# HpWang-whu/RoReg

Measured on AMD Instinct MI355X. Metric: pair-registrations/sec, higher is better.
Workload: dtype f32 (every f32 operand enters the fp16 matrix cores as hi + lo fp16 under a per-keypoint power-of-two block scale: <= 22 significant bits relative to a CONSERVATIVE per-keypoint bound -- measured on the extractor: the bound sits 2^2..2^6 above the keypoint's true coefficient maximum (config.f16x2_sc

## Files before the change

roreg_amd/csrc/fourier.hip:

```cpp
#include "common.h"
#include "primitives.h"
#include <algorithm>
#include <atomic>
#include <cmath>
#include <cstdlib>
#include <type_traits>
#include <utility>
#include <vector>

namespace {

constexpr int NIRR = 5;

struct GemmDescs {
    const float *X[NIRR];
    float *Out[NIRR];
    const float *Add[NIRR];
    const float4 *W[NIRR];
    int K[NIRR], M[NIRR], Mpad[NIRR], N[NIRR];
};

template <int CT>
__global__ __launch_bounds__(256, 2) void irrep_gemm_kernel(GemmDescs p, const int *__restrict__ tiles) {
    extern __shared__ __attribute__((aligned(16))) char smem[];
// ... 1576 lines not shown
    const float *A1, *A2;
    const bf16x8 *A1s, *A2s;
    const f16x8 *A1h, *A2h;
    int f_exp;
    const float *out_bound;
    float *out_rowmax;
    int x_bf16;
    int out_planes;
    int sp_pack;
    float *raw_col;
    int raw_g;
    int B, Bp, C, tiles_per_c, Lout, Lvalid;
    const roreg::LtRow *g_rows;
    const int64_t *g_dr;
    const uint8_t *g_P8;
};

struct QRows { int alpha[64], d[64], i[64]; };
constexpr QRows make_qrows() {
    QRows t{};
    const int dims[NIRR] = {1, 3, 3, 4, 5};
    int off = 0, q = 0;
    for (int r = 0; r < NIRR; ++r) {
        for (int i = 0; i < dims[r]; ++i)
            for (int l = 0; l < dims[r]; ++l, ++q) { t.alpha[q] = off + l * dims[r]; t.d[q] = dims[r]; t.i[q] = i; }
        off += dims[r] * dims[r];
    }
    for (; q < 64; ++q) { t.alpha[q] = 0; t.d[q] = 1; t.i[q] = 0; }
    return t;
}
constexpr QRows kQ = make_qrows();

struct PairSlots {
    int qa[32], qb[32];
    int row[32];
    int i[32];
    int kind[32];
    int d[32];
    int row_alpha[16], row_d[16];
};
constexpr PairSlots make_pair_slots() {
    PairSlots t{};
    const int dims[NIRR] = {1, 3, 3, 4, 5};
    int off = 0, s = 0, row0 = 0;
    for (int r = 0; r < NIRR; ++r) {
        const int d = dims[r];
        for (int l = 0; l < d; ++l) {
            t.row_alpha[row0 + l] = off + l * d; t.row_d[row0 + l] = d;
            for (int i = d % 2; i < d; i += 2, ++s) {
                t.qa[s] = off + i * d + l; t.qb[s] = off + (i + 1) * d + l; t.row[s] = row0 + l; t.i[s] = i; t.kind[s] = 0; t.d[s] = d;
            }
        }
        if (d % 2)
            for (int l = 0; l < d; l += 2, ++s) {
                t.qa[s] = off + l; t.row[s] = row0 + l; t.i[s] = 0; t.d[s] = d;
                if (l + 1 < d) { t.qb[s] = off + l + 1; t.kind[s] = 1; } else { t.qb[s] = 64; t.kind[s] = 2; }
            }
        off += d * d; row0 += d;
    }
    return t;
}
constexpr PairSlots kPS = make_pair_slots();
constexpr int slot_out_q(int m) { const int mm = m & 31, s = (m >> 5) * 16 + (mm & 3) + 4 * (mm >> 3); return (mm & 4) ? kPS.qb[s] : kPS.qa[s]; }

template <int... I, class F>
__device__ __forceinline__ void static_for_impl(std::integer_sequence<int, I...>, F &&f) { (f(std::integral_constant<int, I>{}), ...); }
template <int N, class F>
__device__ __forceinline__ void static_for(F &&f) { static_for_impl(std::make_integer_sequence<int, N>{}, f); }

template <bool IN_SPATIAL, bool OUT_SPATIAL, int SPLIT , int NW , int MINW , bool OUT_ROWS = false, bool GATHER = false >
__global__ __launch_bounds__(NW * 64, MINW) void ft_nonlin_kernel(NonlinParams p) {
    constexpr int NT = NW * 64;
    const int lane = threadIdx.x & 63;
    const int jn = lane & 31, h = lane >> 5;
    const int wave_global = __builtin_amdgcn_readfirstlane((blockIdx.x * NT + threadIdx.x) >> 6);
    const int n_waves = gridDim.x * NW;
    const int B = p.B, C = p.C;
    const int n_tiles = C * p.tiles_per_c;

    constexpr int NPL = SPLIT == 2 ? 2 : 3;
    constexpr int NA1 = SPLIT ? 4 * 2 * NPL * 64 * 4 : 30 * 2 * 64, NA2 = SPLIT ? 4 * 2 * NPL * 64 * 4 : 32 * 2 * 64;
    __shared__ __attribute__((aligned(16))) float sA1[IN_SPATIAL ? 64 : NA1];
    __shared__ __attribute__((aligned(16))) float sA2[OUT_SPATIAL ? 64 : NA2];
    __shared__ float sT[(IN_SPATIAL || OUT_SPATIAL || OUT_ROWS) ? NW * 32 * 65 : 64];
    {
        const float *g1 = SPLIT == 3 ? reinterpret_cast<const float *>(p.A1s) : SPLIT == 2 ? reinterpret_cast<const float *>(p.A1h) : p.A1;
        const float *g2 = SPLIT == 3 ? reinterpret_cast<const float *>(p.A2s) : SPLIT == 2 ? reinterpret_cast<const float *>(p.A2h) : p.A2;
        if (!IN_SPATIAL)
            for (int i = threadIdx.x; i < NA1; i += NT) sA1[i] = g1[i];
        if (!OUT_SPATIAL)
            for (int i = threadIdx.x; i < NA2; i += NT) sA2[i] = g2[i];
    }
    __shared__ float sBias[512], sScale[512], sShift[512];
    __shared__ int sGmap[64];
    if (threadIdx.x < 64) sGmap[threadIdx.x] = (OUT_SPATIAL && p.g_map && threadIdx.x < ROREG_G) ? p.g_map[threadIdx.x] : (int)threadIdx.x;
    __shared__ uint8_t sP8[GATHER ? ROREG_G * ROREG_G : 4];
    if constexpr (GATHER)
        for (int i = threadIdx.x; i < ROREG_G * ROREG_G; i += NT) sP8[i] = p.g_P8[i];
    for (int i = threadIdx.x; i < p.C; i += NT) {
        sBias[i] = (p.bias ? p.bias[i] : 0.f) + (p.bias2 ? p.bias2[i] : 0.f);
        sScale[i] = p.bn_scale ? p.bn_scale[i] : 1.f;
        sShift[i] = p.bn_shift ? p.bn_shift[i] : 0.f;
    }
    __syncthreads();
    const bf16x8 *sA1s = reinterpret_cast<const bf16x8 *>(sA1), *sA2s = reinterpret_cast<const bf16x8 *>(sA2);
    const f16x8 *sA1h = reinterpret_cast<const f16x8 *>(sA1), *sA2h = reinterpret_cast<const f16x8 *>(sA2);
    const size_t Bp = (size_t)p.Bp;
    const size_t hmask = (size_t)0 - (size_t)h;
#define OFF_Q(Q, c, tb) ((size_t)(kQ.alpha[Q] * C + (c) * kQ.d[Q]) * Bp + (size_t)(tb) * (32 * kQ.d[Q]) + kQ.i[Q] * 32)
#define OFF_OF(Q0, Q1, c, tb) (OFF_Q(Q0, c, tb) + ((OFF_Q(Q1, c, tb) - OFF_Q(Q0, c, tb)) & hmask))
    const unsigned lane_next = (unsigned)lane * 4u;
    const unsigned lane_row3 = (unsigned)jn * 4u + (h ? 12u * (unsigned)C * (unsigned)p.Bp : 0u);
    const unsigned lane_row5 = (unsigned)jn * 4u + (h ? 20u * (unsigned)C * (unsigned)p.Bp : 0u);
    auto row_off = [&](auto rc, int c, int tb) -> size_t {
        constexpr int R = decltype(rc)::value;
        return ((size_t)(kPS.row_alpha[R] * C) + (size_t)(c * kPS.row_d[R])) * Bp + (size_t)tb * (32 * kPS.row_d[R]);
    };
    auto slot_ptr = [&](auto sc, const void *buf, int c, int tb) -> const char * {
        constexpr int S = decltype(sc)::value;
        const char *rb = reinterpret_cast<const char *>(buf) + 4 * row_off(std::integral_constant<int, kPS.row[S]>{}, c, tb) + 128 * kPS.i[S];
        return rb + (kPS.kind[S] == 1 ? (kPS.d[S] == 3 ? lane_row3 : lane_row5) : lane_next);
    };

    constexpr int NCV = IN_SPATIAL ? 32 : (SPLIT != 0 ? 32 : 30);
    constexpr bool PACK_OUT = SPLIT == 2 && !OUT_SPATIAL && !OUT_ROWS;
    auto ld_sp = [&](const float *base, size_t i) -> float {
        return p.x_bf16 ? __uint_as_float((unsigned)reinterpret_cast<const unsigned short *>(base)[i] << 16) : base[i];
    };
    float cn[NCV + 1];
    struct GDesc { unsigned lo, hi; int a; };
    auto load_desc = [&](int tile) -> GDesc {
        GDesc d{0u, 0u, 0};
        if constexpr (GATHER) {
            const int c = tile % C, tb = tile / C;
            const int row = min(tb * 32 + jn, B - 1);
            const uint2 w = *reinterpret_cast<const uint2 *>(&p.g_rows[row].src[c >> 5]);
            d.lo = w.x; d.hi = w.y;
            d.a = reinterpret_cast<const int *>(p.g_dr)[2 * (size_t)row];
        }
        return d;
    };
    auto load_rows_gathered = [&](int tile, const GDesc &d, float (&dst)[NCV + 1]) {
        if constexpr (GATHER) {
            const int c = tile % C, tb = tile / C;
            if constexpr (PACK_OUT) dst[NCV] = p.out_bound[tb * 32 + jn];
            const int cg = (c & 31) * ROREG_G, ln = lane < ROREG_G ? lane : 0;
            const bool permuted = !((c >> 5) & 1);
            auto rows = [&](auto bf16c, auto permc) {
                static_for<32>([&](auto ic) {
                    constexpr int i = decltype(ic)::value;
                    const unsigned long long base = ((unsigned long long)(unsigned)__builtin_amdgcn_readlane((int)d.hi, i) << 32) |
                                                    (unsigned)__builtin_amdgcn_readlane((int)d.lo, i);
                    int g = ln;
                    if constexpr (decltype(permc)::value) g = sP8[__builtin_amdgcn_readlane(d.a, i) * ROREG_G + ln];
                    if constexpr (decltype(bf16c)::value)
                        dst[i] = __uint_as_float(lane < ROREG_G ? (unsigned)reinterpret_cast<const unsigned short *>(base)[cg + g] : 0u);
                    else
                        dst[i] = lane < ROREG_G ? reinterpret_cast<const float *>(base)[cg + g] : 0.f;
                });
            };
            using T_ = std::true_type; using F_ = std::false_type;
            if (p.x_bf16) { if (permuted) rows(T_{}, T_{}); else rows(T_{}, F_{}); }
            else { if (permuted) rows(F_{}, T_{}); else rows(F_{}, F_{}); }
        }
    };
    auto load_coefs = [&](int tile, float (&dst)[NCV + 1]) {
        const int c = (IN_SPATIAL || OUT_SPATIAL) ? tile % C : tile / p.tiles_per_c;
        const int tb = (IN_SPATIAL || OUT_SPATIAL) ? tile / C : tile - c * p.tiles_per_c;
        if constexpr (PACK_OUT) dst[NCV] = p.out_bound[tb * 32 + jn];
        if constexpr (OUT_SPATIAL && SPLIT == 2) { if (p.sp_pack) dst[NCV] = p.out_bound[tb * 32 + jn]; }
        if constexpr (IN_SPATIAL) {
            const int b0 = tb * 32;
            if (p.x_bf16) {
                const unsigned short *xs16 = reinterpret_cast<const unsigned short *>(p.x_spatial);
                static_for<32>([&](auto ic) {
                    constexpr int i = decltype(ic)::value;
                    const size_t src = ((size_t)(b0 + i < B ? b0 + i : B - 1) * C + c) * ROREG_G;
                    dst[i] = __uint_as_float(lane < ROREG_G ? (unsigned)xs16[src + lane] : 0u);
                });
            } else {
                static_for<32>([&](auto ic) {
                    constexpr int i = decltype(ic)::value;
                    const size_t src = ((size_t)(b0 + i < B ? b0 + i : B - 1) * C + c) * ROREG_G;
                    dst[i] = lane < ROREG_G ? p.x_spatial[src + lane] : 0.f;
                });
            }
        } else if constexpr (SPLIT != 0) {
            static_for<32>([&](auto ic) {
                constexpr int st = decltype(ic)::value / 8, e = decltype(ic)::value % 8;
                constexpr int q0 = 16 * st + e, q1 = 16 * st + 8 + e;
                if constexpr (q1 < ROREG_G) dst[st * 8 + e] = __builtin_nontemporal_load(p.Xin + OFF_OF(q0, q1, c, tb) + jn);
                else dst[st * 8 + e] = __builtin_nontemporal_load(p.Xin + OFF_Q(q0, c, tb) + jn);
            });
        } else {
            static_for<30>([&](auto ic) {
                constexpr int s = decltype(ic)::value;
                constexpr int q0 = 2 * s, q1 = 2 * s + 1;
                dst[s] = p.Xin[OFF_OF(q0, q1, c, tb) + jn];
            });
        }
    };
    auto mfma6 = [&](const bf16x8 *a, const bf16x8 &b1, const bf16x8 &b2, const bf16x8 &b3, f32x16 c) {
        const bf16x8 a1 = a[0], a2 = a[64], a3 = a[128];
        c = __builtin_amdgcn_mfma_f32_32x32x16_bf16(a3, b1, c, 0, 0, 0);
        c = __builtin_amdgcn_mfma_f32_32x32x16_bf16(a2, b2, c, 0, 0, 0);
        c = __builtin_amdgcn_mfma_f32_32x32x16_bf16(a1, b3, c, 0, 0, 0);
        c = __builtin_amdgcn_mfma_f32_32x32x16_bf16(a2, b1, c, 0, 0, 0);
        c = __builtin_amdgcn_mfma_f32_32x32x16_bf16(a1, b2, c, 0, 0, 0);
        c = __builtin_amdgcn_mfma_f32_32x32x16_bf16(a1, b1, c, 0, 0, 0);
        return c;
    };
    auto mfma3 = [&](const f16x8 *a, const f16x8 &bh, const f16x8 &bl, f32x16 c) {
        const f16x8 ah = a[0], al = a[64];
        c = __builtin_amdgcn_mfma_f32_32x32x16_f16(al, bh, c, 0, 0, 0);
        c = __builtin_amdgcn_mfma_f32_32x32x16_f16(ah, bl, c, 0, 0, 0);
        c = __builtin_amdgcn_mfma_f32_32x32x16_f16(ah, bh, c, 0, 0, 0);
        return c;
    };
    auto column_scale = [&](float mx, float &xscale, float &oscale) {
        mx = fmaxf(mx, __shfl_xor(mx, 32));
        int e = 0;
        if (mx > 0.f && mx < __builtin_inff()) { int ex; (void)frexpf(mx, &ex); e = 14 - ex; }
        xscale = ldexpf(1.f, e); oscale = ldexpf(1.f, -(e + p.f_exp));
    };
    auto process = [&](int tile, int next_tile, float (&cv)[NCV + 1], float (&cnext)[NCV + 1], int next2_tile, const GDesc &dnext, GDesc &dnext2) {
        asm volatile("" ::: "memory");
        const int c = (IN_SPATIAL || OUT_SPATIAL) ? tile % C : tile / p.tiles_per_c;
        const int tbi = (IN_SPATIAL || OUT_SPATIAL) ? tile / C : tile - c * p.tiles_per_c;
        const int b = tbi * 32 + jn;
        const bool valid = b < B;
        const int bb = valid ? b : B - 1;
        f32x16 v[2];
        float wmax = 0.f;
        if (IN_SPATIAL) {
            if constexpr (GATHER) {
                dnext2 = load_desc(next2_tile);
                load_rows_gathered(next_tile, dnext, cnext);
            } else {
                load_coefs(next_tile, cnext);
            }
            __builtin_amdgcn_sched_barrier(0);
            float *ti = sT + (threadIdx.x >> 6) * (32 * 65);
#pragma unroll
            for (int i = 0; i < 32; ++i) ti[i * 65 + lane] = p.x_bf16 ? __uint_as_float(__float_as_uint(cv[i]) << 16) : cv[i];
            asm volatile("s_waitcnt lgkmcnt(0)" ::: "memory");
#pragma unroll
            for (int t = 0; t < 2; ++t)
#pragma unroll
                for (int r = 0; r < 16; ++r) {
                    const int g = t * 32 + (r & 3) + 8 * (r >> 2) + 4 * h;
                    v[t][r] = g < ROREG_G ? ti[jn * 65 + g] : 0.f;
                }
            asm volatile("s_waitcnt lgkmcnt(0)" ::: "memory");
        } else {
            load_coefs(next_tile, cnext);
            __builtin_amdgcn_sched_barrier(0);
#pragma unroll
            for (int t = 0; t < 2; ++t)
#pragma unroll
                for (int r = 0; r < 16; ++r) v[t][r] = 0.f;
            if constexpr (SPLIT == 3) {
#pragma unroll
                for (int st = 0; st < 4; ++st) {
                    float x8[8];
#pragma unroll
                    for (int e = 0; e < 8; ++e) x8[e] = (16 * st + 8 + e < ROREG_G || h == 0) ? cv[st * 8 + e] : 0.f;
                    bf16x8 b1, b2, b3;
                    split3(x8, b1, b2, b3);
                    v[0] = mfma6(sA1s + ((st * 2 + 0) * 3) * 64 + lane, b1, b2, b3, v[0]);
                    v[1] = mfma6(sA1s + ((st * 2 + 1) * 3) * 64 + lane, b1, b2, b3, v[1]);
                }
            } else if constexpr (SPLIT == 2) {
                float mx = 0.f;
#pragma unroll
                for (int s = 0; s < 32; ++s) mx = fmaxf(mx, ((16 * (s >> 3) + 8 + (s & 7) < ROREG_G || h == 0) ? fabsf(cv[s]) : 0.f));
                float xsc, osc;
                column_scale(mx, xsc, osc);
#pragma unroll
                for (int st = 0; st < 4; ++st) {
                    float x8[8];
#pragma unroll
                    for (int e = 0; e < 8; ++e) x8[e] = (16 * st + 8 + e < ROREG_G || h == 0) ? cv[st * 8 + e] : 0.f;
                    f16x8 bh, bl;
                    split2(x8, xsc, bh, bl);
                    v[0] = mfma3(sA1h + ((st * 2 + 0) * 2) * 64 + lane, bh, bl, v[0]);
                    v[1] = mfma3(sA1h + ((st * 2 + 1) * 2) * 64 + lane, bh, bl, v[1]);
                }
#pragma unroll
                for (int t = 0; t < 2; ++t)
#pragma unroll
                    for (int r = 0; r < 16; ++r) v[t][r] *= osc;
            } else {
#pragma unroll
                for (int s = 0; s < 30; ++s) {
                    v[0] = __builtin_amdgcn_mfma_f32_32x32x2f32(sA1[(s * 2 + 0) * 64 + lane], cv[s], v[0], 0, 0, 0);
                    v[1] = __builtin_amdgcn_mfma_f32_32x32x2f32(sA1[(s * 2 + 1) * 64 + lane], cv[s], v[1], 0, 0, 0);
                }
            }
        }
        const float bsum = sBias[c];
        const bool bn = p.bn_scale != nullptr;
        const float sc = sScale[c], sh = sShift[c];
        const bool has_rs = OUT_SPATIAL && p.r_spatial;
        const bool rs_late = has_rs && !bn && !p.g_map && !p.out_rowmax;
        const size_t rs = ((size_t)bb * C + c) * ROREG_G;
        float *tb = (OUT_SPATIAL || OUT_ROWS) ? sT + (threadIdx.x >> 6) * (32 * 65) : nullptr;
        const bool sp_pack = OUT_SPATIAL && SPLIT == 2 && p.sp_pack;
        const float pk_scale = sp_pack ? ldexpf(1.f, bound_exp(cv[NCV])) : 1.f;
#pragma unroll
        for (int t = 0; t < 2; ++t)
#pragma unroll
            for (int r = 0; r < 16; ++r) {
                const int g = t * 32 + (r & 3) + 8 * (r >> 2) + 4 * h;
                float x = v[t][r] + bsum;
                if (OUT_SPATIAL && has_rs && !rs_late && g < ROREG_G) x += ld_sp(p.r_spatial, rs + g);
                if (sp_pack && p.raw_col && g == p.raw_g && valid) p.raw_col[(size_t)bb * C + c] = x;
                if (bn) x = fmaxf(fmaf(x, sc, sh), 0.f);
                if (g >= ROREG_G || !valid) x = 0.f;
                v[t][r] = x;
                if (OUT_SPATIAL && g < ROREG_G) {
                    const int go = sGmap[g];
                    if (go >= 0) {
                        if (sp_pack) {
                            const float xs = x * pk_scale;
                            const _Float16 h1 = (_Float16)xs;
                            const _Float16 l1 = (_Float16)(xs - (float)h1);
                            tb[jn * 65 + go] = __uint_as_float((unsigned)__builtin_bit_cast(unsigned short, h1) | ((unsigned)__builtin_bit_cast(unsigned short, l1) << 16));
                        } else {
                            tb[jn * 65 + go] = x; wmax = fmaxf(wmax, fabsf(x));
                        }
                    }
                }
            }
        if (OUT_SPATIAL) {
            asm volatile("s_waitcnt lgkmcnt(0)" ::: "memory");
            const int b0 = tbi * 32;
            if (b0 + 32 <= B) {
                float *ob = p.out_spatial + ((size_t)b0 * C + c) * p.Lout + lane;
                const size_t ostep = (size_t)C * p.Lout;
                const size_t rb = ((size_t)b0 * C + c) * ROREG_G + (lane < ROREG_G ? lane : 0), rstep = (size_t)C * ROREG_G;
                const unsigned short *r16 = reinterpret_cast<const unsigned short *>(p.r_spatial);
#pragma unroll
                for (int g8 = 0; g8 < 4; ++g8) {
                    float tv[8], rv[8];
#pragma unroll
                    for (int q = 0; q < 8; ++q) tv[q] = tb[(g8 * 8 + q) * 65 + lane];
                    if (rs_late) {
                        if (p.x_bf16) {
#pragma unroll
                            for (int q = 0; q < 8; ++q) rv[q] = __uint_as_float((unsigned)r16[rb + (size_t)(g8 * 8 + q) * rstep]);
#pragma unroll
                            for (int q = 0; q < 8; ++q) tv[q] += __uint_as_float(__float_as_uint(rv[q]) << 16);
                        } else {
#pragma unroll
                            for (int q = 0; q < 8; ++q) rv[q] = p.r_spatial[rb + (size_t)(g8 * 8 + q) * rstep];
#pragma unroll
                            for (int q = 0; q < 8; ++q) tv[q] += rv[q];
                        }
                    }
#pragma unroll
                    for (int q = 0; q < 8; ++q)
                        if (lane < p.Lout) ob[(size_t)(g8 * 8 + q) * ostep] = lane < p.Lvalid ? tv[q] : 0.f;
                }
            } else {
                for (int bl = 0; bl < 32 && b0 + bl < B; ++bl)
                    if (lane < p.Lout) {
                        float tv = tb[bl * 65 + lane];
                        if (rs_late && lane < ROREG_G) tv += ld_sp(p.r_spatial, ((size_t)(b0 + bl) * C + c) * ROREG_G + lane);
                        p.out_spatial[((size_t)(b0 + bl) * C + c) * p.Lout + lane] = lane < p.Lvalid ? tv : 0.f;
                    }
            }
            asm volatile("s_waitcnt lgkmcnt(0)" ::: "memory");
            if (p.out_rowmax) {
                wmax = fmaxf(wmax, __shfl_xor(wmax, 32));
                atomicMax(reinterpret_cast<unsigned *>(p.out_rowmax) + bb, __float_as_uint(valid ? wmax : 0.f));
            }
        }
        if (!OUT_SPATIAL) {
            f32x16 o[2];
#pragma unroll
            for (int t = 0; t < 2; ++t)
#pragma unroll
                for (int r = 0; r < 16; ++r) o[t][r] = 0.f;
            if constexpr (SPLIT == 3) {
#pragma unroll
                for (int st = 0; st < 4; ++st) {
                    float x8[8];
#pragma unroll
                    for (int e = 0; e < 8; ++e) x8[e] = v[st >> 1][8 * (st & 1) + e];
                    bf16x8 b1, b2, b3;
                    split3(x8, b1, b2, b3);
                    o[0] = mfma6(sA2s + ((st * 2 + 0) * 3) * 64 + lane, b1, b2, b3, o[0]);
                    o[1] = mfma6(sA2s + ((st * 2 + 1) * 3) * 64 + lane, b1, b2, b3, o[1]);
                }
            } else if constexpr (SPLIT == 2) {
                float mx = 0.f;
#pragma unroll
                for (int t = 0; t < 2; ++t)
#pragma unroll
                    for (int r = 0; r < 16; ++r) mx = fmaxf(mx, fabsf(v[t][r]));
                float xsc, osc;
                column_scale(mx, xsc, osc);
#pragma unroll
                for (int st = 0; st < 4; ++st) {
                    float x8[8];
#pragma unroll
                    for (int e = 0; e < 8; ++e) x8[e] = v[st >> 1][8 * (st & 1) + e];
                    f16x8 bh, bl;
                    split2(x8, xsc, bh, bl);
                    o[0] = mfma3(sA2h + ((st * 2 + 0) * 2) * 64 + lane, bh, bl, o[0]);
                    o[1] = mfma3(sA2h + ((st * 2 + 1) * 2) * 64 + lane, bh, bl, o[1]);
                }
                if constexpr (PACK_OUT) {
                    const float psc = osc * ldexpf(1.f, bound_exp(cv[NCV]));
#pragma unroll
                    for (int t = 0; t < 2; ++t)
#pragma unroll
                        for (int r = 0; r < 16; ++r) {
                            const float x = o[t][r] * psc;
                            const _Float16 h1 = (_Float16)x;
                            const _Float16 l1 = (_Float16)(x - (float)h1);
                            o[t][r] = __uint_as_float((unsigned)__builtin_bit_cast(unsigned short, h1) | ((unsigned)__builtin_bit_cast(unsigned short, l1) << 16));
                        }
                } else {
#pragma unroll
                    for (int t = 0; t < 2; ++t)
#pragma unroll
                        for (int r = 0; r < 16; ++r) o[t][r] *= osc;
                }
            } else {
#pragma unroll
                for (int t = 0; t < 2; ++t)
#pragma unroll
                    for (int r = 0; r < 16; ++r) {
                        const int s = t * 16 + r;
                        o[0] = __builtin_amdgcn_mfma_f32_32x32x2f32(sA2[(s * 2 + 0) * 64 + lane], v[t][r], o[0], 0, 0, 0);
                        o[1] = __builtin_amdgcn_mfma_f32_32x32x2f32(sA2[(s * 2 + 1) * 64 + lane], v[t][r], o[1], 0, 0, 0);
                    }
            }
            if constexpr (OUT_ROWS) {
#pragma unroll
                for (int t = 0; t < 2; ++t)
#pragma unroll
                    for (int r = 0; r < 16; ++r) {
                        const int qq = h ? kPS.qb[t * 16 + r] : kPS.qa[t * 16 + r];
                        if (qq < ROREG_G) tb[jn * 65 + qq] = o[t][r];
                    }
                asm volatile("s_waitcnt lgkmcnt(0)" ::: "memory");
                const int b0 = tbi * 32;
                if (b0 + 32 <= B) {
                    float *ob = p.out_spatial + ((size_t)b0 * C + c) * ROREG_G + lane;
                    const size_t ostep = (size_t)C * ROREG_G;
#pragma unroll
                    for (int g8 = 0; g8 < 4; ++g8) {
                        float tv[8];
#pragma unroll
                        for (int q = 0; q < 8; ++q) tv[q] = tb[(g8 * 8 + q) * 65 + lane];
#pragma unroll
                        for (int q = 0; q < 8; ++q)
                            if (lane < ROREG_G) ob[(size_t)(g8 * 8 + q) * ostep] = tv[q];
                    }
                } else {
                    for (int bl = 0; bl < 32 && b0 + bl < B; ++bl)
                        if (lane < ROREG_G) p.out_spatial[((size_t)(b0 + bl) * C + c) * ROREG_G + lane] = tb[bl * 65 + lane];
                }
                asm volatile("s_waitcnt lgkmcnt(0)" ::: "memory");
            } else if (PACK_OUT && p.out_planes) {
                const int tb = tbi;
                const unsigned sel = (jn & 16) ? 0x07060302u : 0x05040100u;
                static_for<32>([&](auto ic) {
                    constexpr int S = decltype(ic)::value, t = S / 16, r = S % 16;
                    const unsigned own = __float_as_uint(o[t][r]);
                    const auto pr = __builtin_amdgcn_permlane16_swap(own, own, false, false);
                    const unsigned word = __builtin_amdgcn_perm(pr[1], pr[0], sel);
                    unsigned *dst = reinterpret_cast<unsigned *>(const_cast<char *>(slot_ptr(ic, p.Xout, c, tb)));
                    if (kPS.kind[S] != 2 || h == 0) __builtin_nontemporal_store(word, dst);
                });
            } else {
                const int tb = tbi;
                static_for<32>([&](auto ic) {
                    constexpr int S = decltype(ic)::value, t = S / 16, r = S % 16;
                    float *dst = reinterpret_cast<float *>(const_cast<char *>(slot_ptr(ic, p.Xout, c, tb)));
                    if (kPS.kind[S] != 2 || h == 0) __builtin_nontemporal_store(o[t][r], dst);
                });
            }
        }
    };
    if (wave_global < n_tiles) {
        const int last = wave_global + ((n_tiles - 1 - wave_global) / n_waves) * n_waves;
        float cb[NCV + 1];
        GDesc da{0u, 0u, 0}, db{0u, 0u, 0};
        if constexpr (GATHER) {
            da = load_desc(wave_global);
            db = load_desc(min(wave_global + n_waves, last));
            load_rows_gathered(wave_global, da, cn);
        } else {
            load_coefs(wave_global, cn);
        }
        __builtin_amdgcn_s_waitcnt(0x0F70);
        for (int tile = wave_global; tile <= last; tile += 2 * n_waves) {
            const int t1 = min(tile + n_waves, last), t2 = min(tile + 2 * n_waves, last), t3 = min(tile + 3 * n_waves, last);
            process(tile, t1, cn, cb, t2, db, da);
            process(t1, t2, cb, cn, t3, da, db);
        }
    }
}

#undef OFF_OF
#undef OFF_Q

float *g_A1 = nullptr, *g_A2 = nullptr;
uint16_t *g_A1s = nullptr, *g_A2s = nullptr, *g_A1h = nullptr, *g_A2h = nullptr;
int g_f_exp = 0;

}

extern "C" int roreg_set_fourier_tables(const float *F_host ) {
    ROREG_REQUIRE(F_host, "roreg_set_fourier_tables: null table");
    static float A1[30 * 2 * 64], A2[32 * 2 * 64];
    for (int s = 0; s < 30; ++s)
        for (int tile = 0; tile < 2; ++tile)
            for (int lane = 0; lane < 64; ++lane) {
                const int qq = 2 * s + (lane >> 5), g = tile * 32 + (lane & 31);
                A1[(s * 2 + tile) * 64 + lane] = g < 60 ? F_host[qq * 60 + g] : 0.f;
            }
    for (int t = 0; t < 2; ++t)
        for (int r = 0; r < 16; ++r)
            for (int tile = 0; tile < 2; ++tile)
                for (int lane = 0; lane < 64; ++lane) {
                    const int qq = slot_out_q(tile * 32 + (lane & 31)), g = t * 32 + (r & 3) + 8 * (r >> 2) + 4 * (lane >> 5);
                    A2[((t * 16 + r) * 2 + tile) * 64 + lane] = (qq < 60 && g < 60) ? F_host[qq * 60 + g] : 0.f;
                }
    if (!g_A1) {
        if (hipMalloc(&g_A1, sizeof(A1)) != hipSuccess || hipMalloc(&g_A2, sizeof(A2)) != hipSuccess) {
            roreg::set_error("roreg_set_fourier_tables: hipMalloc failed");
            return 1;
        }
    }
    if (hipMemcpy(g_A1, A1, sizeof(A1), hipMemcpyHostToDevice) != hipSuccess || hipMemcpy(g_A2, A2, sizeof(A2), hipMemcpyHostToDevice) != hipSuccess) {
        roreg::set_error("roreg_set_fourier_tables: hipMemcpy failed");
        return 1;
    }
    static uint16_t A1s[4 * 2 * 3 * 64 * 8], A2s[4 * 2 * 3 * 64 * 8];
    auto split3_host = [](float x, uint16_t out[3]) {
        float rem = x;
        for (int sp = 0; sp < 3; ++sp) {
            uint32_t u; memcpy(&u, &rem, 4);
            const uint32_t r = ((u >> 16) & 1u) + 0x7fffu;
            const uint16_t hi = (uint16_t)((u + r) >> 16);
// ... 293 lines not shown
    float mx = 0.f, m1 = 0.f, m0 = 0.f;
    if (b < B) {
        const size_t row = (size_t)b * ROREG_F * ROREG_G;
        for (int i = lane; i < ROREG_F * ROREG_G; i += 64) {
            const float v = x_bf16 ? __uint_as_float((unsigned)reinterpret_cast<const unsigned short *>(x)[row + i] << 16) : x[row + i];
            const int c = i / ROREG_G;
            mx = fmaxf(mx, fabsf(v));
            m1 = fmaxf(m1, fmaxf(fmaf(v, role_scale[c], role_shift[c]), 0.f));
            m0 = fmaxf(m0, fmaxf(fmaf(v, role_scale[ROREG_F + c], role_shift[ROREG_F + c]), 0.f));
        }
#pragma unroll
        for (int o = 32; o > 0; o >>= 1) { mx = fmaxf(mx, __shfl_xor(mx, o)); m1 = fmaxf(m1, __shfl_xor(m1, o)); m0 = fmaxf(m0, __shfl_xor(m0, o)); }
        if (lane == 0) { role_out[(size_t)b * 4] = m1; role_out[(size_t)b * 4 + 1] = m0; }
    }
    if (lane == 0) bound[b] = mx * 7.7536f;
}

extern "C" int roreg_row_bound_roles(const void *x_spatial, int x_bf16, float *bound_out, const float *role_scale, const float *role_shift, float *role_out,
                                     int B, void *stream) {
    ROREG_REQUIRE(x_spatial && bound_out && role_scale && role_shift && role_out && B > 0, "roreg_row_bound_roles: bad arguments");
    const int Bp = (B + 31) / 32 * 32;
    hipLaunchKernelGGL(row_bound_roles_kernel, dim3((Bp + 3) / 4), dim3(256), 0, roreg::as_stream(stream), reinterpret_cast<const float *>(x_spatial), x_bf16, bound_out,
                       B, Bp, role_scale, role_shift, role_out);
    ROREG_CHECK_LAUNCH("roreg_row_bound_roles");
    return 0;
}

extern "C" int roreg_row_bound(const void *x_spatial, int x_bf16, const float *bn_scale, const float *bn_shift, float *bound_out, int B, int C,
                               void *stream) {
    ROREG_REQUIRE(x_spatial && bound_out && B > 0 && C > 0, "roreg_row_bound: bad arguments");
    ROREG_REQUIRE((bn_scale == nullptr) == (bn_shift == nullptr), "roreg_row_bound: bn_scale and bn_shift go together");
    const int Bp = (B + 31) / 32 * 32;
    hipLaunchKernelGGL(row_bound_kernel, dim3((Bp + 3) / 4), dim3(256), 0, roreg::as_stream(stream), reinterpret_cast<const float *>(x_spatial), x_bf16, bn_scale, bn_shift,
                       bound_out, B, Bp, C);
    ROREG_CHECK_LAUNCH("roreg_row_bound");
    return 0;
}

template <void (*KERN)(NonlinParams)>
static void launch_ft(const NonlinParams &p, long long n_tiles, hipStream_t s) {
    static const int resident = [] {
        int per_cu = 0, dev = 0, cus = 256;
        if (hipOccupancyMaxActiveBlocksPerMultiprocessor(&per_cu, KERN, 256, 0) != hipSuccess || per_cu < 1) per_cu = 2;
        if (hipGetDevice(&dev) == hipSuccess) (void)hipDeviceGetAttribute(&cus, hipDeviceAttributeMultiprocessorCount, dev);
        return per_cu * cus;
    }();
    static const int rounds = [] { const char *e = getenv("ROREG_FT_ROUNDS"); const int r = e ? atoi(e) : 0; return r > 0 ? r : 4; }();
    const long long want = (n_tiles + 3) / 4, cap = (long long)resident * rounds;
    hipLaunchKernelGGL(KERN, dim3((unsigned)(want > cap ? cap : want)), dim3(256), 0, s, p);
}

extern "C" int roreg_ft_nonlin(const float *Xin, const float *x_spatial, const float *bias, const float *bias2,
                               const float *bn_scale, const float *bn_shift, const float *resid_spatial, float *Xout, float *out_spatial,
                               const int32_t *g_map, int Lout, int Lvalid, int B, int C, int split, const float *out_bound, float *out_rowmax,
                               int spatial_bf16, int out_planes, void *stream) {
    ROREG_REQUIRE(g_A1 && g_A2, "roreg_ft_nonlin: roreg_set_fourier_tables has not been called");
    ROREG_REQUIRE((Xin != nullptr) != (x_spatial != nullptr), "roreg_ft_nonlin: exactly one of Xin / x_spatial");
    ROREG_REQUIRE((Xout != nullptr) != (out_spatial != nullptr), "roreg_ft_nonlin: exactly one of Xout / out_spatial");
    ROREG_REQUIRE((bn_scale == nullptr) == (bn_shift == nullptr) && B > 0 && C > 0 && C <= 512, "roreg_ft_nonlin: bad arguments (C <= 512)");
    ROREG_REQUIRE((long long)60 * C * B < (1ll << 40), "roreg_ft_nonlin: tensor too large");
    ROREG_REQUIRE(!g_map || (Lout >= Lvalid && Lvalid > 0 && Lout <= 64), "roreg_ft_nonlin: bad Lout/Lvalid");
    NonlinParams p;
    memset(&p, 0, sizeof(p));
    p.Xin = Xin; p.Xout = Xout;
    p.x_spatial = x_spatial; p.r_spatial = resid_spatial; p.out_spatial = out_spatial;
    p.g_map = g_map; p.Lout = g_map ? Lout : ROREG_G; p.Lvalid = g_map ? Lvalid : ROREG_G;
    p.bias = bias; p.bias2 = bias2; p.bn_scale = bn_scale; p.bn_shift = bn_shift; p.A1 = g_A1; p.A2 = g_A2;
    p.A1s = reinterpret_cast<const bf16x8 *>(g_A1s); p.A2s = reinterpret_cast<const bf16x8 *>(g_A2s); p.out_bound = out_bound; p.out_rowmax = out_rowmax; p.x_bf16 = spatial_bf16;
    p.A1h = reinterpret_cast<const f16x8 *>(g_A1h); p.A2h = reinterpret_cast<const f16x8 *>(g_A2h); p.f_exp = g_f_exp;
    p.B = B; p.Bp = (B + 31) / 32 * 32; p.C = C; p.tiles_per_c = (B + 31) / 32;
    p.out_planes = out_planes;
    ROREG_REQUIRE((unsigned long long)C * p.Bp * 20ull < (1ull << 32), "roreg_ft_nonlin: C * round_up(B, 32) must stay below 2^32 / 20 (32-bit lane offsets)");
    ROREG_REQUIRE(!out_planes || (split == 2 && Xout), "roreg_ft_nonlin: out_planes is a layout of the fp16 x 2 coefficient output");
    const long long n_tiles = (long long)C * p.tiles_per_c;
    hipStream_t s = roreg::as_stream(stream);
    roreg::ProfScope prof(roreg::PROF_FT_NONLIN, s);
    const bool in_sp = x_spatial != nullptr, out_sp = out_spatial != nullptr;
    if (in_sp && out_sp) { roreg::set_error("roreg_ft_nonlin: spatial -> spatial is not a transform"); return 2; }
    ROREG_REQUIRE(split != 2 || out_sp || out_bound, "roreg_ft_nonlin: split = 2 writes the coefficients as fp16 hi/lo pairs and needs out_bound");
    ROREG_REQUIRE(!spatial_bf16 || in_sp || resid_spatial, "roreg_ft_nonlin: spatial_bf16 refers to x_spatial / resid_spatial");
    ROREG_REQUIRE(!out_rowmax || out_sp, "roreg_ft_nonlin: out_rowmax goes with a group-domain output");
    ROREG_REQUIRE(split >= 0 && split <= 2, "roreg_ft_nonlin: split must be 0 (f32 MFMA), 1 (bf16 x 3) or 2 (fp16 x 2)");
    if (split == 2) {
        if (in_sp) launch_ft<ft_nonlin_kernel<true, false, 2, 4, 1>>(p, n_tiles, s);
        else if (!out_sp) launch_ft<ft_nonlin_kernel<false, false, 2, 4, 1>>(p, n_tiles, s);
        else launch_ft<ft_nonlin_kernel<false, true, 2, 4, 1>>(p, n_tiles, s);
    } else if (split == 1) {
        if (in_sp) launch_ft<ft_nonlin_kernel<true, false, 3, 4, 1>>(p, n_tiles, s);
        else if (!out_sp) launch_ft<ft_nonlin_kernel<false, false, 3, 4, 1>>(p, n_tiles, s);
        else launch_ft<ft_nonlin_kernel<false, true, 3, 4, 1>>(p, n_tiles, s);
    } else {
        if (in_sp) launch_ft<ft_nonlin_kernel<true, false, 0, 4, 1>>(p, n_tiles, s);
        else if (!out_sp) launch_ft<ft_nonlin_kernel<false, false, 0, 4, 1>>(p, n_tiles, s);
        else launch_ft<ft_nonlin_kernel<false, true, 0, 4, 1>>(p, n_tiles, s);
    }
    ROREG_CHECK_LAUNCH("roreg_ft_nonlin");
    return 0;
}

extern "C" int roreg_ft_nonlin_packed(const float *Xin, const float *bias, const float *bn_scale, const float *bn_shift, uint32_t *out_words,
                                      const int32_t *g_map, int Lout, int Lvalid, int B, int C, const float *out_bound, float *raw_col, int raw_g,
                                      void *stream) {
    ROREG_REQUIRE(g_A1 && g_A2, "roreg_ft_nonlin_packed: roreg_set_fourier_tables has not been called");
    ROREG_REQUIRE(Xin && out_words && out_bound && B > 0 && C > 0 && C <= 512 && (bn_scale == nullptr) == (bn_shift == nullptr), "roreg_ft_nonlin_packed: bad arguments");
    ROREG_REQUIRE(!g_map || (Lout >= Lvalid && Lvalid > 0 && Lout <= 64), "roreg_ft_nonlin_packed: bad Lout/Lvalid");
    ROREG_REQUIRE(!raw_col || (raw_g >= 0 && raw_g < ROREG_G), "roreg_ft_nonlin_packed: raw_g out of range");
    NonlinParams p;
    memset(&p, 0, sizeof(p));
    p.Xin = Xin; p.out_spatial = reinterpret_cast<float *>(out_words);
    p.g_map = g_map; p.Lout = g_map ? Lout : ROREG_G; p.Lvalid = g_map ? Lvalid : ROREG_G;
    p.bias = bias; p.bn_scale = bn_scale; p.bn_shift = bn_shift; p.A1 = g_A1; p.A2 = g_A2;
    p.A1s = reinterpret_cast<const bf16x8 *>(g_A1s); p.A2s = reinterpret_cast<const bf16x8 *>(g_A2s);
    p.A1h = reinterpret_cast<const f16x8 *>(g_A1h); p.A2h = reinterpret_cast<const f16x8 *>(g_A2h); p.f_exp = g_f_exp;
    p.out_bound = out_bound; p.sp_pack = 1; p.raw_col = raw_col; p.raw_g = raw_g;
    p.B = B; p.Bp = (B + 31) / 32 * 32; p.C = C; p.tiles_per_c = (B + 31) / 32;
    ROREG_REQUIRE((unsigned long long)C * p.Bp * 20ull < (1ull << 32), "roreg_ft_nonlin_packed: C * round_up(B, 32) must stay below 2^32 / 20 (32-bit lane offsets)");
    hipStream_t s = roreg::as_stream(stream);
    roreg::ProfScope prof(roreg::PROF_FT_NONLIN, s);
    launch_ft<ft_nonlin_kernel<false, true, 2, 4, 1>>(p, (long long)C * p.tiles_per_c, s);
    ROREG_CHECK_LAUNCH("roreg_ft_nonlin_packed");
    return 0;
}

extern "C" int roreg_ft_nonlin_gathered(const uint64_t *rows, const int64_t *dr, int feat_bf16, const float *bn_scale, const float *bn_shift, float *Xout,
                                        int B, const float *out_bound, int out_planes, void *stream) {
    ROREG_REQUIRE(g_A1 && g_A2, "roreg_ft_nonlin_gathered: roreg_set_fourier_tables has not been called");
    ROREG_REQUIRE(roreg::group_tables().ready, "roreg_ft_nonlin_gathered: group tables not set");
    ROREG_REQUIRE(rows && dr && Xout && out_bound && B > 0 && (bn_scale == nullptr) == (bn_shift == nullptr), "roreg_ft_nonlin_gathered: bad arguments");
    constexpr int C = 4 * ROREG_F;
    ROREG_REQUIRE((long long)60 * C * B < (1ll << 40), "roreg_ft_nonlin_gathered: tensor too large");
    NonlinParams p;
    memset(&p, 0, sizeof(p));
    p.Xout = Xout; p.Lout = ROREG_G; p.Lvalid = ROREG_G;
    p.bn_scale = bn_scale; p.bn_shift = bn_shift; p.A1 = g_A1; p.A2 = g_A2;
    p.A1s = reinterpret_cast<const bf16x8 *>(g_A1s); p.A2s = reinterpret_cast<const bf16x8 *>(g_A2s);
    p.A1h = reinterpret_cast<const f16x8 *>(g_A1h); p.A2h = reinterpret_cast<const f16x8 *>(g_A2h); p.f_exp = g_f_exp;
    p.out_bound = out_bound; p.x_bf16 = feat_bf16; p.out_planes = out_planes;
    p.g_rows = reinterpret_cast<const roreg::LtRow *>(rows); p.g_dr = dr; p.g_P8 = roreg::group_tables().P8;
    p.B = B; p.Bp = (B + 31) / 32 * 32; p.C = C; p.tiles_per_c = (B + 31) / 32;
    ROREG_REQUIRE((unsigned long long)C * p.Bp * 20ull < (1ull << 32), "roreg_ft_nonlin_gathered: 128 * round_up(B, 32) must stay below 2^32 / 20 (32-bit lane offsets)");
    hipStream_t s = roreg::as_stream(stream);
    roreg::ProfScope prof(roreg::PROF_FT_NONLIN, s);
    launch_ft<ft_nonlin_kernel<true, false, 2, 4, 1, false, true>>(p, (long long)C * p.tiles_per_c, s);
    ROREG_CHECK_LAUNCH("roreg_ft_nonlin_gathered");
    return 0;
}

extern "C" int roreg_feat_coefs(const void *x, int x_bf16, float *out, int B, int C, int split, void *stream) {
    if (B == 0) return 0;
    ROREG_REQUIRE(g_A1 && g_A2, "roreg_feat_coefs: roreg_set_fourier_tables has not been called");
    ROREG_REQUIRE(x && out && B > 0 && C > 0 && C <= 512 && split >= 0 && split <= 2, "roreg_feat_coefs: bad arguments");
    NonlinParams p;
    memset(&p, 0, sizeof(p));
    p.x_spatial = reinterpret_cast<const float *>(x); p.x_bf16 = x_bf16; p.out_spatial = out;
    p.Lout = ROREG_G; p.Lvalid = ROREG_G; p.A1 = g_A1; p.A2 = g_A2;
    p.A1s = reinterpret_cast<const bf16x8 *>(g_A1s); p.A2s = reinterpret_cast<const bf16x8 *>(g_A2s);
    p.A1h = reinterpret_cast<const f16x8 *>(g_A1h); p.A2h = reinterpret_cast<const f16x8 *>(g_A2h); p.f_exp = g_f_exp;
    p.B = B; p.Bp = (B + 31) / 32 * 32; p.C = C; p.tiles_per_c = (B + 31) / 32;
    const long long n_tiles = (long long)C * p.tiles_per_c;
    hipStream_t s = roreg::as_stream(stream);
    if (split == 2) launch_ft<ft_nonlin_kernel<true, false, 2, 4, 1, true>>(p, n_tiles, s);
    else if (split == 1) launch_ft<ft_nonlin_kernel<true, false, 3, 4, 1, true>>(p, n_tiles, s);
    else launch_ft<ft_nonlin_kernel<true, false, 0, 4, 1, true>>(p, n_tiles, s);
    ROREG_CHECK_LAUNCH("roreg_feat_coefs");
    return 0;
}
```

Measured before the change: 1124.

## Halve nonlinearity transpose scratch to two 16-row rounds and raise min waves

The per-wave LDS transpose buffer in the Fourier nonlinearity kernel shrinks from 32 rows to 16 for non-gather, non-row-output variants. The transpose into and out of the group domain now runs in two rounds, with each half of the lanes reading or writing its 16 rows per round. Output values are buffered in registers before the staged store, and the raw-column write is deferred until after the loop. Launch bounds for the fp16x2 spatial-input and spatial-output variants are raised to 3 minimum waves per EU, so more blocks fit per CU. The cost is extra LDS round-trips and waits, and higher register pressure from the buffered values under a tighter register cap.

```diff
diff --git a/roreg_amd/csrc/fourier.hip b/roreg_amd/csrc/fourier.hip
--- a/roreg_amd/csrc/fourier.hip
+++ b/roreg_amd/csrc/fourier.hip
@@ -1682,7 +1682,8 @@
     constexpr int NA1 = SPLIT ? 4 * 2 * NPL * 64 * 4 : 30 * 2 * 64, NA2 = SPLIT ? 4 * 2 * NPL * 64 * 4 : 32 * 2 * 64;
     __shared__ __attribute__((aligned(16))) float sA1[IN_SPATIAL ? 64 : NA1];
     __shared__ __attribute__((aligned(16))) float sA2[OUT_SPATIAL ? 64 : NA2];
-    __shared__ float sT[(IN_SPATIAL || OUT_SPATIAL || OUT_ROWS) ? NW * 32 * 65 : 64];
+    constexpr int TK = (GATHER || OUT_ROWS) ? 32 : 16, NRND = 32 / TK;
+    __shared__ float sT[(IN_SPATIAL || OUT_SPATIAL || OUT_ROWS) ? NW * TK * 65 : 64];
     {
         const float *g1 = SPLIT == 3 ? reinterpret_cast<const float *>(p.A1s) : SPLIT == 2 ? reinterpret_cast<const float *>(p.A1h) : p.A1;
         const float *g2 = SPLIT == 3 ? reinterpret_cast<const float *>(p.A2s) : SPLIT == 2 ? reinterpret_cast<const float *>(p.A2h) : p.A2;
@@ -1840,18 +1841,27 @@
                 load_coefs(next_tile, cnext);
             }
             __builtin_amdgcn_sched_barrier(0);
-            float *ti = sT + (threadIdx.x >> 6) * (32 * 65);
-#pragma unroll
-            for (int i = 0; i < 32; ++i) ti[i * 65 + lane] = p.x_bf16 ? __uint_as_float(__float_as_uint(cv[i]) << 16) : cv[i];
-            asm volatile("s_waitcnt lgkmcnt(0)" ::: "memory");
+            float *ti = sT + (threadIdx.x >> 6) * (TK * 65);
 #pragma unroll
             for (int t = 0; t < 2; ++t)
 #pragma unroll
-                for (int r = 0; r < 16; ++r) {
-                    const int g = t * 32 + (r & 3) + 8 * (r >> 2) + 4 * h;
-                    v[t][r] = g < ROREG_G ? ti[jn * 65 + g] : 0.f;
+                for (int r = 0; r < 16; ++r) v[t][r] = 0.f;
+#pragma unroll
+            for (int k = 0; k < NRND; ++k) {
+#pragma unroll
+                for (int i = 0; i < TK; ++i) ti[i * 65 + lane] = p.x_bf16 ? __uint_as_float(__float_as_uint(cv[k * TK + i]) << 16) : cv[k * TK + i];
+                asm volatile("s_waitcnt lgkmcnt(0)" ::: "memory");
+                if (NRND == 1 || (jn >> 4) == k) {
+#pragma unroll
+                    for (int t = 0; t < 2; ++t)
+#pragma unroll
+                        for (int r = 0; r < 16; ++r) {
+                            const int g = t * 32 + (r & 3) + 8 * (r >> 2) + 4 * h;
+                            v[t][r] = g < ROREG_G ? ti[(jn & (TK - 1)) * 65 + g] : 0.f;
+                        }
                 }
-            asm volatile("s_waitcnt lgkmcnt(0)" ::: "memory");
+                asm volatile("s_waitcnt lgkmcnt(0)" ::: "memory");
+            }
         } else {
             load_coefs(next_tile, cnext);
             __builtin_amdgcn_sched_barrier(0);
@@ -1904,7 +1914,10 @@
         const bool has_rs = OUT_SPATIAL && p.r_spatial;
         const bool rs_late = has_rs && !bn && !p.g_map && !p.out_rowmax;
         const size_t rs = ((size_t)bb * C + c) * ROREG_G;
-        float *tb = (OUT_SPATIAL || OUT_ROWS) ? sT + (threadIdx.x >> 6) * (32 * 65) : nullptr;
+        float *tb = (OUT_SPATIAL || OUT_ROWS) ? sT + (threadIdx.x >> 6) * (TK * 65) : nullptr;
+        float wv[2][16];
+        float rawx = 0.f;
+        bool raw_hit = false;
         const bool sp_pack = OUT_SPATIAL && SPLIT == 2 && p.sp_pack;
         const float pk_scale = sp_pack ? ldexpf(1.f, bound_exp(cv[NCV])) : 1.f;
 #pragma unroll
@@ -1914,34 +1927,49 @@
                 const int g = t * 32 + (r & 3) + 8 * (r >> 2) + 4 * h;
                 float x = v[t][r] + bsum;
                 if (OUT_SPATIAL && has_rs && !rs_late && g < ROREG_G) x += ld_sp(p.r_spatial, rs + g);
-                if (sp_pack && p.raw_col && g == p.raw_g && valid) p.raw_col[(size_t)bb * C + c] = x;
+                if (sp_pack && g == p.raw_g) { rawx = x; raw_hit = true; }
                 if (bn) x = fmaxf(fmaf(x, sc, sh), 0.f);
                 if (g >= ROREG_G || !valid) x = 0.f;
                 v[t][r] = x;
-                if (OUT_SPATIAL && g < ROREG_G) {
-                    const int go = sGmap[g];
-                    if (go >= 0) {
-                        if (sp_pack) {
-                            const float xs = x * pk_scale;
-                            const _Float16 h1 = (_Float16)xs;
-                            const _Float16 l1 = (_Float16)(xs - (float)h1);
-                            tb[jn * 65 + go] = __uint_as_float((unsigned)__builtin_bit_cast(unsigned short, h1) | ((unsigned)__builtin_bit_cast(unsigned short, l1) << 16));
-                        } else {
-                            tb[jn * 65 + go] = x; wmax = fmaxf(wmax, fabsf(x));
+                if (OUT_SPATIAL) {
+                    if (sp_pack) {
+                        const float xs = x * pk_scale;
+                        const _Float16 h1 = (_Float16)xs;
+                        const _Float16 l1 = (_Float16)(xs - (float)h1);
+                        wv[t][r] = __uint_as_float((unsigned)__builtin_bit_cast(unsigned short, h1) | ((unsigned)__builtin_bit_cast(unsigned short, l1) << 16));
+                    } else {
+                        wv[t][r] = x;
+                    }
+                }
+            }
+        if (OUT_SPATIAL && sp_pack && p.raw_col && raw_hit && valid) p.raw_col[(size_t)bb * C + c] = rawx;
+        if (OUT_SPATIAL) {
+            const int b0 = tbi * 32;
+#pragma unroll
+            for (int k = 0; k < NRND; ++k) {
+            if (NRND == 1 || (jn >> 4) == k) {
+#pragma unroll
+                for (int t = 0; t < 2; ++t)
+#pragma unroll
+                    for (int r = 0; r < 16; ++r) {
+                        const int g = t * 32 + (r & 3) + 8 * (r >> 2) + 4 * h;
+                        if (g < ROREG_G) {
+                            const int go = sGmap[g];
+                            if (go >= 0) {
+                                tb[(jn & (TK - 1)) * 65 + go] = wv[t][r];
+                                if (!sp_pack) wmax = fmaxf(wmax, fabsf(wv[t][r]));
+                            }
                         }
                     }
-                }
-            }
-        if (OUT_SPATIAL) {
+            }
             asm volatile("s_waitcnt lgkmcnt(0)" ::: "memory");
-            const int b0 = tbi * 32;
             if (b0 + 32 <= B) {
-                float *ob = p.out_spatial + ((size_t)b0 * C + c) * p.Lout + lane;
                 const size_t ostep = (size_t)C * p.Lout;
-                const size_t rb = ((size_t)b0 * C + c) * ROREG_G + (lane < ROREG_G ? lane : 0), rstep = (size_t)C * ROREG_G;
+                float *ob = p.out_spatial + ((size_t)b0 * C + c) * p.Lout + lane + (size_t)(k * TK) * ostep;
+                const size_t rstep = (size_t)C * ROREG_G, rb = ((size_t)b0 * C + c) * ROREG_G + (lane < ROREG_G ? lane : 0) + (size_t)(k * TK) * rstep;
                 const unsigned short *r16 = reinterpret_cast<const unsigned short *>(p.r_spatial);
 #pragma unroll
-                for (int g8 = 0; g8 < 4; ++g8) {
+                for (int g8 = 0; g8 < TK / 8; ++g8) {
                     float tv[8], rv[8];
 #pragma unroll
                     for (int q = 0; q < 8; ++q) tv[q] = tb[(g8 * 8 + q) * 65 + lane];
@@ -1963,14 +1991,15 @@
                         if (lane < p.Lout) ob[(size_t)(g8 * 8 + q) * ostep] = lane < p.Lvalid ? tv[q] : 0.f;
                 }
             } else {
-                for (int bl = 0; bl < 32 && b0 + bl < B; ++bl)
+                for (int bl = k * TK; bl < (k + 1) * TK && b0 + bl < B; ++bl)
                     if (lane < p.Lout) {
-                        float tv = tb[bl * 65 + lane];
+                        float tv = tb[(bl - k * TK) * 65 + lane];
                         if (rs_late && lane < ROREG_G) tv += ld_sp(p.r_spatial, ((size_t)(b0 + bl) * C + c) * ROREG_G + lane);
                         p.out_spatial[((size_t)(b0 + bl) * C + c) * p.Lout + lane] = lane < p.Lvalid ? tv : 0.f;
                     }
             }
             asm volatile("s_waitcnt lgkmcnt(0)" ::: "memory");
+            }
             if (p.out_rowmax) {
                 wmax = fmaxf(wmax, __shfl_xor(wmax, 32));
                 atomicMax(reinterpret_cast<unsigned *>(p.out_rowmax) + bb, __float_as_uint(valid ? wmax : 0.f));
@@ -2039,20 +2068,24 @@
                     }
             }
             if constexpr (OUT_ROWS) {
-#pragma unroll
-                for (int t = 0; t < 2; ++t)
-#pragma unroll
-                    for (int r = 0; r < 16; ++r) {
-                        const int qq = h ? kPS.qb[t * 16 + r] : kPS.qa[t * 16 + r];
-                        if (qq < ROREG_G) tb[jn * 65 + qq] = o[t][r];
-                    }
+                const int b0 = tbi * 32;
+#pragma unroll
+                for (int k = 0; k < NRND; ++k) {
+                if (NRND == 1 || (jn >> 4) == k) {
+#pragma unroll
+                    for (int t = 0; t < 2; ++t)
+#pragma unroll
+                        for (int r = 0; r < 16; ++r) {
+                            const int qq = h ? kPS.qb[t * 16 + r] : kPS.qa[t * 16 + r];
+                            if (qq < ROREG_G) tb[(jn & (TK - 1)) * 65 + qq] = o[t][r];
+                        }
+                }
                 asm volatile("s_waitcnt lgkmcnt(0)" ::: "memory");
-                const int b0 = tbi * 32;
                 if (b0 + 32 <= B) {
-                    float *ob = p.out_spatial + ((size_t)b0 * C + c) * ROREG_G + lane;
                     const size_t ostep = (size_t)C * ROREG_G;
-#pragma unroll
-                    for (int g8 = 0; g8 < 4; ++g8) {
+                    float *ob = p.out_spatial + ((size_t)b0 * C + c) * ROREG_G + lane + (size_t)(k * TK) * ostep;
+#pragma unroll
+                    for (int g8 = 0; g8 < TK / 8; ++g8) {
                         float tv[8];
 #pragma unroll
                         for (int q = 0; q < 8; ++q) tv[q] = tb[(g8 * 8 + q) * 65 + lane];
@@ -2061,10 +2094,11 @@
                             if (lane < ROREG_G) ob[(size_t)(g8 * 8 + q) * ostep] = tv[q];
                     }
                 } else {
-                    for (int bl = 0; bl < 32 && b0 + bl < B; ++bl)
-                        if (lane < ROREG_G) p.out_spatial[((size_t)(b0 + bl) * C + c) * ROREG_G + lane] = tb[bl * 65 + lane];
+                    for (int bl = k * TK; bl < (k + 1) * TK && b0 + bl < B; ++bl)
+                        if (lane < ROREG_G) p.out_spatial[((size_t)(b0 + bl) * C + c) * ROREG_G + lane] = tb[(bl - k * TK) * 65 + lane];
                 }
                 asm volatile("s_waitcnt lgkmcnt(0)" ::: "memory");
+                }
             } else if (PACK_OUT && p.out_planes) {
                 const int tb = tbi;
                 const unsigned sel = (jn & 16) ? 0x07060302u : 0x05040100u;
@@ -2524,9 +2558,9 @@
     ROREG_REQUIRE(!out_rowmax || out_sp, "roreg_ft_nonlin: out_rowmax goes with a group-domain output");
     ROREG_REQUIRE(split >= 0 && split <= 2, "roreg_ft_nonlin: split must be 0 (f32 MFMA), 1 (bf16 x 3) or 2 (fp16 x 2)");
     if (split == 2) {
-        if (in_sp) launch_ft<ft_nonlin_kernel<true, false, 2, 4, 1>>(p, n_tiles, s);
+        if (in_sp) launch_ft<ft_nonlin_kernel<true, false, 2, 4, 3>>(p, n_tiles, s);
         else if (!out_sp) launch_ft<ft_nonlin_kernel<false, false, 2, 4, 1>>(p, n_tiles, s);
-        else launch_ft<ft_nonlin_kernel<false, true, 2, 4, 1>>(p, n_tiles, s);
+        else launch_ft<ft_nonlin_kernel<false, true, 2, 4, 3>>(p, n_tiles, s);
     } else if (split == 1) {
         if (in_sp) launch_ft<ft_nonlin_kernel<true, false, 3, 4, 1>>(p, n_tiles, s);
         else if (!out_sp) launch_ft<ft_nonlin_kernel<false, false, 3, 4, 1>>(p, n_tiles, s);
@@ -2559,7 +2593,7 @@
     ROREG_REQUIRE((unsigned long long)C * p.Bp * 20ull < (1ull << 32), "roreg_ft_nonlin_packed: C * round_up(B, 32) must stay below 2^32 / 20 (32-bit lane offsets)");
     hipStream_t s = roreg::as_stream(stream);
     roreg::ProfScope prof(roreg::PROF_FT_NONLIN, s);
-    launch_ft<ft_nonlin_kernel<false, true, 2, 4, 1>>(p, (long long)C * p.tiles_per_c, s);
+    launch_ft<ft_nonlin_kernel<false, true, 2, 4, 3>>(p, (long long)C * p.tiles_per_c, s);
     ROREG_CHECK_LAUNCH("roreg_ft_nonlin_packed");
     return 0;
 }
```

Result: no change. 1130 (median of 6 runs) (+0.6%).
